# AIM-SE/AC-TSR

Hardware: NVIDIA B200
Metric: AC-SASRec train seq/s (higher is better)
Workload: dtype f32

## Files before the change

ac-tsr_b200/csrc/dense_fwd.cu:

```cuda
#include "acsr_common.cuh"
#include "../../include/acsr.h"

namespace acsr {

constexpr int kDfThreads = 352;
constexpr int kDfD = 64;
constexpr int kDfBM = 128;
constexpr int kDfOpFloats = 64 * 64;
constexpr int kDfBlkBytes = 2 * kDfOpFloats * 4;
constexpr int kDfMaxI = 256;

struct DfParams {
  const float* ctx; const float* res; long long rows, res_rows; int I, act, passes;
  const float* ops;
  const float *bo, *lnA_w, *lnA_b, *b1, *b2, *lnF_w, *lnF_b;
  float epsA, epsF, p_drop;
  const float *mask_a, *mask_f; const RngState* rng; uint32_t stream_a, stream_f;
  float *hz, *st_a, *h, *z1, *a1, *z2, *st_f, *out;
  int m_tiles;
};

__global__ void __launch_bounds__(256) dense_prep_kernel(const float* __restrict__ Wo, const float* __restrict__ W1,
                                                         const float* __restrict__ W2, int I, float* __restrict__ ops) {
  pdl_wait();
  const int nc = I / 64, blk = blockIdx.x;
  float* hi = ops + (long long)blk * 2 * kDfOpFloats;
  float* lo = hi + kDfOpFloats;
  for (int e = threadIdx.x; e < 64 * 16; e += blockDim.x) {
    const int n = e >> 4, kc = e & 15;
    const float* src;
    if (blk == 0) src = Wo + n * 64 + kc * 4;
    else if (blk <= nc) src = W1 + (long long)((blk - 1) * 64 + n) * 64 + kc * 4;
    else src = W2 + (long long)n * I + (blk - 1 - nc) * 64 + kc * 4;
    const float4 x = *reinterpret_cast<const float4*>(src);
    const float4 h4 = make_float4(to_tf32(x.x), to_tf32(x.y), to_tf32(x.z), to_tf32(x.w));
    const int off = kc * 256 + n * 4;
    *reinterpret_cast<float4*>(hi + off) = h4;
    *reinterpret_cast<float4*>(lo + off) = make_float4(x.x - h4.x, x.y - h4.y, x.z - h4.z, x.w - h4.w);
  }
}

struct DfCfg {
  static constexpr int kOffWo = 0;
  static constexpr int kOffW1 = kOffWo + kDfBlkBytes;
  static constexpr int kOffW2 = kOffW1 + 2 * kDfBlkBytes;
  static constexpr int kOffPar = kOffW2 + 2 * kDfBlkBytes;
  static constexpr int kParFloats = 6 * 64 + kDfMaxI;
  static constexpr int kOffBar = kOffPar + kParFloats * 4;
  static constexpr int kNumBars = 24;
  static constexpr int kSmemBytes = kOffBar + kNumBars * 8 + 16;
  static constexpr int kColAcc = 0, kColA = 64, kColC = 192, kColL = 320;
};

__device__ __forceinline__ float df_drop(const DfParams& p, const float* mask, uint32_t stream, long long row, int q, float* m4) {
  if (mask != nullptr) {
    const float4 mm = __ldg(reinterpret_cast<const float4*>(mask + row * kDfD + q * 4));
    m4[0] = mm.x; m4[1] = mm.y; m4[2] = mm.z; m4[3] = mm.w;
  } else if (p.p_drop > 0.f && p.rng != nullptr) {
    const float inv_keep = 1.0f / (1.0f - p.p_drop);
    const uint4 w = philox4x32(p.rng->seed, p.rng->step, stream, (unsigned long long)row * 16 + q);
    m4[0] = drop_mult(w.x, p.p_drop, inv_keep); m4[1] = drop_mult(w.y, p.p_drop, inv_keep);
    m4[2] = drop_mult(w.z, p.p_drop, inv_keep); m4[3] = drop_mult(w.w, p.p_drop, inv_keep);
  } else {
    m4[0] = m4[1] = m4[2] = m4[3] = 1.0f;
  }
  return 0.f;
}

__global__ void __launch_bounds__(kDfThreads, 1) dense_fwd_kernel(const DfParams p) {
  using Cfg = DfCfg;
  extern __shared__ __align__(128) uint8_t smem[];
  const int warp = threadIdx.x >> 5, lane = threadIdx.x & 31;
  const int nc = p.I / 64;
  float* sPar = reinterpret_cast<float*>(smem + Cfg::kOffPar);
  float *s_bo = sPar, *s_b2 = sPar + 64, *s_lnAw = sPar + 128, *s_lnAb = sPar + 192, *s_lnFw = sPar + 256, *s_lnFb = sPar + 320,
        *s_b1 = sPar + 384;
  uint64_t* bars = reinterpret_cast<uint64_t*>(smem + Cfg::kOffBar);
  uint64_t* wo_full = bars;
  uint64_t* w1_full = bars + 1;
  uint64_t* w1_empty = bars + 3;
  uint64_t* w2_full = bars + 5;
  uint64_t* w2_empty = bars + 7;
  uint64_t* a_full = bars + 9;
  uint64_t* s1_full = bars + 10;
  uint64_t* h_full = bars + 11;
  uint64_t* c_full = bars + 12;
  uint64_t* a_ready = bars + 14;
  uint64_t* c_empty = bars + 16;
  uint64_t* s3_full = bars + 18;
  uint64_t* tile_done = bars + 19;
  uint32_t* tmem_slot = reinterpret_cast<uint32_t*>(bars + Cfg::kNumBars);

  pdl_launch_dependents();
  if (threadIdx.x == 0) {
    mbar_init(wo_full, 1);
    for (int s = 0; s < 2; ++s) {
      mbar_init(w1_full + s, 1); mbar_init(w1_empty + s, 1); mbar_init(w2_full + s, 1); mbar_init(w2_empty + s, 1);
      mbar_init(c_full + s, 1); mbar_init(a_ready + s, 256); mbar_init(c_empty + s, 1);
    }
    mbar_init(a_full, 128); mbar_init(s1_full, 1); mbar_init(h_full, 128); mbar_init(s3_full, 1); mbar_init(tile_done, 128);
    mbar_fence_init();
  }
  if (warp == 1) tmem_alloc<512>(tmem_slot);
  for (int i = threadIdx.x; i < 64; i += kDfThreads) {
    s_bo[i] = p.bo[i]; s_b2[i] = p.b2[i]; s_lnAw[i] = p.lnA_w[i]; s_lnAb[i] = p.lnA_b[i]; s_lnFw[i] = p.lnF_w[i]; s_lnFb[i] = p.lnF_b[i];
  }
  for (int i = threadIdx.x; i < p.I; i += kDfThreads) s_b1[i] = p.b1[i];
  tc_fence_before();
  __syncthreads();
  tc_fence_after();
  const uint32_t tmem_base = *tmem_slot;
  const int my_tiles = (int)blockIdx.x < p.m_tiles ? (p.m_tiles - (int)blockIdx.x + (int)gridDim.x - 1) / (int)gridDim.x : 0;

  if (warp == 0) {
    if (lane == 0 && my_tiles > 0) {
      mbar_arrive_expect_tx(wo_full, kDfBlkBytes);
      bulk_g2s(smem + Cfg::kOffWo, p.ops, kDfBlkBytes, wo_full);
      for (int it = 0; it < my_tiles; ++it)
        for (int c = 0; c < nc; ++c) {
          const int g = it * nc + c, b = g & 1;
          const uint32_t ph = (g >> 1) & 1;
          mbar_wait(w1_empty + b, ph ^ 1);
          mbar_arrive_expect_tx(w1_full + b, kDfBlkBytes);
          bulk_g2s(smem + Cfg::kOffW1 + b * kDfBlkBytes, p.ops + (long long)(1 + c) * 2 * kDfOpFloats, kDfBlkBytes, w1_full + b);
          mbar_wait(w2_empty + b, ph ^ 1);
          mbar_arrive_expect_tx(w2_full + b, kDfBlkBytes);
          bulk_g2s(smem + Cfg::kOffW2 + b * kDfBlkBytes, p.ops + (long long)(1 + nc + c) * 2 * kDfOpFloats, kDfBlkBytes, w2_full + b);
        }
    }
  } else if (warp == 1 || warp == 2) {
    if (lane == 0 && my_tiles > 0) {
      const uint32_t idesc = umma_idesc_tf32(kDfBM, 64);
      constexpr uint32_t kLbo = 64 * 16, kSbo = 128;
      const int npass = p.passes == 3 ? 3 : 1;
      const uint32_t a_hi = tmem_base + Cfg::kColA, a_lo = a_hi + 64;
      auto mma24 = [&](uint32_t d_tmem, uint32_t ahi, uint32_t alo, uint32_t bsm, bool first_zero) {
        uint32_t acc = first_zero ? 0u : 1u;
        for (int ps = 0; ps < npass; ++ps) {
          const uint32_t a_base = (npass == 3 && ps == 0) ? alo : ahi;
          const uint32_t b_base = bsm + ((npass == 3 && ps == 1) ? kDfOpFloats * 4 : 0);
#pragma unroll
          for (int ks = 0; ks < 8; ++ks) {
            umma_tf32_ts(d_tmem, a_base + ks * 8, umma_desc_kmajor(b_base + ks * 2 * kLbo, kLbo, kSbo), idesc, acc);
            acc = 1;
          }
        }
      };
      if (warp == 1) {
        mbar_wait(wo_full, 0);
        for (int it = 0; it < my_tiles; ++it) {
          mbar_wait(a_full, it & 1);
          tc_fence_after();
          mma24(tmem_base + Cfg::kColAcc, a_hi, a_lo, smem_u32(smem + Cfg::kOffWo), true);
          umma_commit(s1_full);
          mbar_wait(h_full, it & 1);
          for (int c = 0; c < nc; ++c) {
            const int g = it * nc + c, b = g & 1;
            const uint32_t ph = (g >> 1) & 1;
            mbar_wait(w1_full + b, ph);
            mbar_wait(c_empty + b, ph ^ 1);
            tc_fence_after();
            mma24(tmem_base + Cfg::kColC + b * 64, a_hi, a_lo, smem_u32(smem + Cfg::kOffW1 + b * kDfBlkBytes), true);
            umma_commit(w1_empty + b);
            umma_commit(c_full + b);
          }
        }
      } else {
        for (int it = 0; it < my_tiles; ++it) {
          for (int c = 0; c < nc; ++c) {
            const int g = it * nc + c, b = g & 1;
            const uint32_t ph = (g >> 1) & 1;
            mbar_wait(a_ready + b, ph);
            mbar_wait(w2_full + b, ph);
            tc_fence_after();
            mma24(tmem_base + Cfg::kColAcc, tmem_base + Cfg::kColC + b * 64, tmem_base + Cfg::kColL + b * 64,
                  smem_u32(smem + Cfg::kOffW2 + b * kDfBlkBytes), c == 0);
            umma_commit(w2_empty + b);
            umma_commit(c_empty + b);
          }
          umma_commit(s3_full);
        }
      }
    }
  } else if (warp < 11) {
    pdl_wait();
    const int quarter = warp & 3;
    const int half = (warp - 3) >> 2;
    const int row = quarter * 32 + lane;
    const uint32_t t_lane = tmem_base + ((uint32_t)(quarter * 32) << 16);
    for (int it = 0; it < my_tiles; ++it) {
      const long long grow = (long long)(blockIdx.x + it * gridDim.x) * kDfBM + row;
      const bool row_ok = grow < p.rows;
      if (half == 1) {
        float4 cx[16];
#pragma unroll
        for (int q = 0; q < 16; ++q)
          cx[q] = row_ok ? __ldg(reinterpret_cast<const float4*>(p.ctx + grow * kDfD + q * 4)) : make_float4(0.f, 0.f, 0.f, 0.f);
        mbar_wait(tile_done, (it & 1) ^ 1);
        tc_fence_after();
#pragma unroll
        for (int hcol = 0; hcol < 2; ++hcol) {
          float hi[32], lo[32];
#pragma unroll
          for (int q = 0; q < 8; ++q) {
            const float4 v = cx[hcol * 8 + q];
            hi[4 * q] = to_tf32(v.x); hi[4 * q + 1] = to_tf32(v.y); hi[4 * q + 2] = to_tf32(v.z); hi[4 * q + 3] = to_tf32(v.w);
            lo[4 * q] = v.x - hi[4 * q]; lo[4 * q + 1] = v.y - hi[4 * q + 1]; lo[4 * q + 2] = v.z - hi[4 * q + 2]; lo[4 * q + 3] = v.w - hi[4 * q + 3];
          }
          tmem_st32(t_lane + Cfg::kColA + hcol * 32, hi);
          tmem_st32(t_lane + Cfg::kColA + 64 + hcol * 32, lo);
        }
        tc_fence_before();
        mbar_arrive(a_full);
      }
      if (half == 0) {
        mbar_wait(s1_full, it & 1);
        tc_fence_after();
        float x[64];
        tmem_ld32(t_lane + Cfg::kColAcc, x);
        tmem_ld32(t_lane + Cfg::kColAcc + 32, x + 32);
        float s = 0.f;
        if (row_ok) {
          float* hz = p.hz + grow * kDfD;
#pragma unroll
          for (int i = 0; i < 64; i += 4) *reinterpret_cast<float4*>(hz + i) = make_float4(x[i], x[i + 1], x[i + 2], x[i + 3]);
          const float* rr = p.res + (grow % p.res_rows) * kDfD;
#pragma unroll
          for (int q = 0; q < 16; ++q) {
            float m4[4];
            df_drop(p, p.mask_a, p.stream_a, grow, q, m4);
            const float4 r4 = __ldg(reinterpret_cast<const float4*>(rr + q * 4));
            const float rv[4] = {r4.x, r4.y, r4.z, r4.w};
#pragma unroll
            for (int v = 0; v < 4; ++v) {
              const int c = q * 4 + v;
              x[c] = (x[c] + s_bo[c]) * m4[v] + rv[v];
              s += x[c];
            }
          }
        } else {
#pragma unroll
          for (int c = 0; c < 64; ++c) x[c] = 0.f;
        }
        const float mean = s * (1.0f / 64);
        float var = 0.f;
#pragma unroll
        for (int c = 0; c < 64; ++c) { const float t = x[c] - mean; var = fmaf(t, t, var); }
        const float rstd = 1.0f / sqrtf(var * (1.0f / 64) + p.epsA);
#pragma unroll
        for (int c = 0; c < 64; ++c) x[c] = row_ok ? (x[c] - mean) * rstd * s_lnAw[c] + s_lnAb[c] : 0.f;
        if (row_ok) {
          float* ho = p.h + grow * kDfD;
#pragma unroll
          for (int c = 0; c < 64; c += 4) *reinterpret_cast<float4*>(ho + c) = make_float4(x[c], x[c + 1], x[c + 2], x[c + 3]);
          p.st_a[2 * grow] = mean; p.st_a[2 * grow + 1] = rstd;
        }
#pragma unroll
        for (int hcol = 0; hcol < 2; ++hcol) {
          float hi[32], lo[32];
#pragma unroll
          for (int i = 0; i < 32; ++i) { hi[i] = to_tf32(x[hcol * 32 + i]); lo[i] = x[hcol * 32 + i] - hi[i]; }
          tmem_st32(t_lane + Cfg::kColA + hcol * 32, hi);
          tmem_st32(t_lane + Cfg::kColA + 64 + hcol * 32, lo);
        }
        tc_fence_before();
        mbar_arrive(h_full);
      }
      for (int c = 0; c < nc; ++c) {
        const int g = it * nc + c, b = g & 1;
        const uint32_t ph = (g >> 1) & 1;
        mbar_wait(c_full + b, ph);
        tc_fence_after();
        float v[32], lo[32];
        tmem_ld32(t_lane + Cfg::kColC + b * 64 + half * 32, v);
        const int col0 = c * 64 + half * 32;
        if (row_ok) {
          float* z = p.z1 + grow * p.I + col0;
#pragma unroll
          for (int i = 0; i < 32; i += 4) *reinterpret_cast<float4*>(z + i) = make_float4(v[i], v[i + 1], v[i + 2], v[i + 3]);
        }
#pragma unroll
        for (int i = 0; i < 32; ++i) v[i] = row_ok ? act_fwd(p.act, v[i] + s_b1[col0 + i]) : 0.f;
        if (row_ok) {
          float* a = p.a1 + grow * p.I + col0;
#pragma unroll
          for (int i = 0; i < 32; i += 4) *reinterpret_cast<float4*>(a + i) = make_float4(v[i], v[i + 1], v[i + 2], v[i + 3]);
        }
#pragma unroll
        for (int i = 0; i < 32; ++i) { const float hi = to_tf32(v[i]); lo[i] = v[i] - hi; v[i] = hi; }
        tmem_st32(t_lane + Cfg::kColC + b * 64 + half * 32, v);
        tmem_st32(t_lane + Cfg::kColL + b * 64 + half * 32, lo);
        tc_fence_before();
        mbar_arrive(a_ready + b);
      }
      if (half == 0) {
        mbar_wait(s3_full, it & 1);
        tc_fence_after();
        float x[64];
        tmem_ld32(t_lane + Cfg::kColAcc, x);
        tmem_ld32(t_lane + Cfg::kColAcc + 32, x + 32);
        if (row_ok) {
          float* z = p.z2 + grow * kDfD;
#pragma unroll
          for (int i = 0; i < 64; i += 4) *reinterpret_cast<float4*>(z + i) = make_float4(x[i], x[i + 1], x[i + 2], x[i + 3]);
        }
        float s = 0.f;
#pragma unroll
        for (int hcol = 0; hcol < 2; ++hcol) {
          float hi[32], lo[32];
          tmem_ld32(t_lane + Cfg::kColA + hcol * 32, hi);
          tmem_ld32(t_lane + Cfg::kColA + 64 + hcol * 32, lo);
#pragma unroll
          for (int q = 0; q < 8; ++q) {
            float m4[4] = {1.f, 1.f, 1.f, 1.f};
            if (row_ok) df_drop(p, p.mask_f, p.stream_f, grow, hcol * 8 + q, m4);
#pragma unroll
            for (int v = 0; v < 4; ++v) {
              const int i = q * 4 + v, c = hcol * 32 + i;
              x[c] = (x[c] + s_b2[c]) * m4[v] + (hi[i] + lo[i]);
              s += x[c];
            }
          }
        }
        tc_fence_before();
        mbar_arrive(tile_done);
        const float mean = s * (1.0f / 64);
        float var = 0.f;
#pragma unroll
        for (int c = 0; c < 64; ++c) { const float t = x[c] - mean; var = fmaf(t, t, var); }
        const float rstd = 1.0f / sqrtf(var * (1.0f / 64) + p.epsF);
        if (row_ok) {
          float* o = p.out + grow * kDfD;
#pragma unroll
          for (int c = 0; c < 64; c += 4)
            *reinterpret_cast<float4*>(o + c) = make_float4((x[c] - mean) * rstd * s_lnFw[c] + s_lnFb[c], (x[c + 1] - mean) * rstd * s_lnFw[c + 1] + s_lnFb[c + 1],
                                                            (x[c + 2] - mean) * rstd * s_lnFw[c + 2] + s_lnFb[c + 2], (x[c + 3] - mean) * rstd * s_lnFw[c + 3] + s_lnFb[c + 3]);
          p.st_f[2 * grow] = mean; p.st_f[2 * grow + 1] = rstd;
        }
      }
    }
  }
  tc_fence_before();
  __syncthreads();
  if (warp == 1) {
    tc_fence_after();
    tmem_dealloc<512>(tmem_base);
  }
}

}

using namespace acsr;

extern "C" {

int64_t acsr_dense_prep_floats(int I) { return (I > 0 && I % 64 == 0) ? (int64_t)(1 + 2 * (I / 64)) * 2 * kDfOpFloats : 0; }

int acsr_dense_prep(const float* Wo, const float* W1, const float* W2, int d, int I, float* ops, void* stream) {
  if (d != kDfD || I <= 0 || I > kDfMaxI || (I & 63)) {
    set_error("dense_prep: hidden size %d / inner size %d unsupported (64; multiples of 64 up to %d)", d, I, kDfMaxI);
    return ACSR_ERR_UNSUPPORTED;
  }
  ACSR_REQUIRE(Wo && W1 && W2 && ops, "dense_prep: NULL pointer");
  launch_pdl(dense_prep_kernel, dim3(1 + 2 * (I / 64)), dim3(256), 0, (cudaStream_t)stream, Wo, W1, W2, I, ops);
  return check_launch("dense_prep");
}

int acsr_dense_fwd(const float* ctx, const float* res, int64_t rows, int64_t res_rows, int d, int I, int act, const float* ops,
                   const float* bo, const float* lnA_w, const float* lnA_b, float epsA, const float* b1, const float* b2,
                   const float* lnF_w, const float* lnF_b, float epsF, float p_drop, const float* mask_a, const float* mask_f,
                   const void* rng, uint32_t stream_a, uint32_t stream_f, float* hz, float* st_a, float* h, float* z1, float* a1,
                   float* z2, float* st_f, float* out, int passes, void* stream) {
  if (d != kDfD || I <= 0 || I > kDfMaxI || (I & 63)) {
    set_error("dense_fwd: hidden size %d / inner size %d unsupported (64; multiples of 64 up to %d)", d, I, kDfMaxI);
    return ACSR_ERR_UNSUPPORTED;
  }
  ACSR_REQUIRE(ctx && res && ops && bo && lnA_w && lnA_b && b1 && b2 && lnF_w && lnF_b, "dense_fwd: NULL input");
  ACSR_REQUIRE(hz && st_a && h && z1 && a1 && z2 && st_f && out, "dense_fwd: NULL output");
  ACSR_REQUIRE(rows >= 0 && res_rows > 0 && act >= 0 && act <= 4, "dense_fwd: bad sizes");
  ACSR_REQUIRE(passes == 1 || passes == 3, "dense_fwd: passes must be 1 or 3");
  ACSR_REQUIRE(p_drop >= 0.f && p_drop < 1.f, "dense_fwd: dropout p=%f", p_drop);
  ACSR_REQUIRE(!(p_drop > 0.f && rng == nullptr && (mask_a == nullptr || mask_f == nullptr)), "dense_fwd: p>0 needs masks or rng");
  if (rows == 0) return ACSR_OK;
  DfParams p = {};
  p.ctx = ctx; p.res = res; p.rows = rows; p.res_rows = res_rows; p.I = I; p.act = act; p.passes = passes; p.ops = ops;
  p.bo = bo; p.lnA_w = lnA_w; p.lnA_b = lnA_b; p.b1 = b1; p.b2 = b2; p.lnF_w = lnF_w; p.lnF_b = lnF_b;
  p.epsA = epsA; p.epsF = epsF; p.p_drop = p_drop; p.mask_a = mask_a; p.mask_f = mask_f; p.rng = (const RngState*)rng;
  p.stream_a = stream_a; p.stream_f = stream_f;
  p.hz = hz; p.st_a = st_a; p.h = h; p.z1 = z1; p.a1 = a1; p.z2 = z2; p.st_f = st_f; p.out = out;
  p.m_tiles = (int)((rows + kDfBM - 1) / kDfBM);
  static_assert(DfCfg::kSmemBytes <= 227 * 1024, "shared memory budget");
  cudaError_t e = cudaFuncSetAttribute(dense_fwd_kernel, cudaFuncAttributeMaxDynamicSharedMemorySize, DfCfg::kSmemBytes);
  if (e != cudaSuccess) { set_error("dense_fwd: smem attr: %s", cudaGetErrorString(e)); return ACSR_ERR_CUDA; }
  const int grid = p.m_tiles < kNumSMs ? p.m_tiles : kNumSMs;
  launch_pdl(dense_fwd_kernel, dim3(grid), dim3(kDfThreads), DfCfg::kSmemBytes, (cudaStream_t)stream, p);
  return check_launch("dense_fwd");
}

}
```

ac-tsr_b200/fused_step.py:

```python
import math

import torch

from . import ops
from ._lib import LIB
from .ops import _p, _stream


class _RandSlice(object):

    def __init__(self, rand, sl):
        self.rand, self.sl = rand, sl

    def get(self, key):
        t = self.rand.get(key)
        return None if t is None else t[self.sl].contiguous()


class FusedTrainStep(object):
    def __init__(self, model, optimizer):
        if model.loss_type not in ('CE', 'BPR'):
            raise NotImplementedError("Make sure 'loss_type' in ['BPR', 'CE']!")
        self.m, self.opt = model, optimizer
        self.buf = {}
        self.vp = None
        self.tc = (bool(getattr(model, 'tc_linear', True)) and model.hidden_size == 64 and model.inner_size <= 256
                   and model.inner_size % 4 == 0)
        self.tc_wgrad = bool(getattr(model, 'tc_wgrad', True))
        self.passes = 3
        self.overlap_wgrad = bool(getattr(model, 'overlap_wgrad', True))
        self.n_branches = int(getattr(model, 'step_branches', 1))
        self._streams = {}
        self.compact_last = bool(getattr(model, 'compact_last', True))
        import os
        self.order_side = os.environ.get('ACSR_ORDER_SIDE', '1') == '1'
        self.fold_attack = os.environ.get('ACSR_FOLD_ATTACK', '1') == '1'
        self.fold_gate = os.environ.get('ACSR_FOLD_GATE', '0') == '1'
        self.pdl = bool(getattr(model, 'pdl', True))
        self.tail_fused = (self.tc and model.inner_size % 16 == 0 and os.environ.get('ACSR_TAIL_FUSED', '1') == '1')
        self.fuse_act_bwd = os.environ.get('ACSR_FUSE_ACT_BWD', '0') == '1'
        self.dense_fused = (self.tc and model.inner_size % 64 == 0 and os.environ.get('ACSR_DENSE_FUSED', '0') == '1')
        self.dense_bwd = (self.tc and model.inner_size % 64 == 0 and os.environ.get('ACSR_DENSE_BWD', '1') == '1')
        self.split_wgrad = int(os.environ.get('ACSR_SPLIT_WGRAD', '1'))
        self.ce_fused_bwd = model.hidden_size == 64 and os.environ.get('ACSR_CE_FUSED_BWD', '1') == '1'

    def _stream_for(self, dev, key):
        if key not in self._streams:
            self._streams[key] = torch.cuda.Stream(device=dev)
        return self._streams[key]

    def _branch_buffers(self, Bs, L, dev, idx, grads=True):
        key = ('branch', Bs, L, idx)
        if key in self.buf:
            return self.buf[key]
        m = self.m
        d, I, N = m.hidden_size, m.inner_size, m.n_layers
        T = Bs * L

        def f(*s):
            return torch.empty(s, dtype=torch.float32, device=dev)
        b = dict(T=T, x0=f(T, d), st_e=f(T, 2), layers=[], order=torch.empty(Bs, dtype=torch.int32, device=dev))
        for l in range(N):
            R = 2 * T if l == N - 1 else T
            qkv5 = f(6, T, d)
            qkv, aqk = qkv5[:3], qkv5[3:5]
            Rp = 1 if (l == N - 1 and self.compact_last) else R
            lb = dict(qkv5=qkv5, qkv=qkv, aqk=aqk, mq=qkv[0], mk=qkv[1], mv=qkv[2], aq=aqk[0], ak=aqk[1],
                      gl=(qkv5[5].view(-1)[:T * L].view(T, L) if L <= d else f(T, L)), ctx=f(R, d),
                      hz=f(Rp, d), st_a=f(Rp, 2), h=f(Rp, d), z1=f(Rp, I), a1=f(Rp, I), z2=f(Rp, d), st_f=f(Rp, 2), out=f(Rp, d))
            if grads:
                for n, w in (('d_z2', d), ('d_z1', I), ('d_hz', d), ('d_gl', L)):
                    lb[n] = f(2 * T if (Rp > 1 or n == 'd_gl') else 1, w)
                lb['d_qkv'], lb['d_aqk'] = f(3, 2 * T, d), f(2, 2 * T, d)
                lb['d_mq'], lb['d_mk'], lb['d_mv'] = lb['d_qkv'][0], lb['d_qkv'][1], lb['d_qkv'][2]
                lb['d_aq'], lb['d_ak'] = lb['d_aqk'][0], lb['d_aqk'][1]
            b['layers'].append(lb)
        C = 2 * Bs
        b['c'] = dict(ctx=f(C, d), x=f(Bs, d), hz=f(C, d), st_a=f(C, 2), h=f(C, d), z1=f(C, I), a1=f(C, I), z2=f(C, d), st_f=f(C, 2),
                      out=f(C, d), d_out=f(C, d), d_z2=f(C, d), d_h=f(C, d), d_a1=f(C, I), d_z1=f(C, I), d_hz=f(C, d), d_x=f(C, d),
                      d_ctx=f(C, d))
        if grads:
            for n, w in (('d_out', d), ('d_a1', I), ('d_h', d), ('d_x', d), ('d_ctx', d)):
                b[n] = f(2 * T, w)
        self.buf[key] = b
        return b

    def _joint_buffers(self, B, dev):
        key = ('joint', B)
        if key in self.buf:
            return self.buf[key]
        m = self.m
        d, N, V = m.hidden_size, m.n_layers, m.n_items

        def f(*s):
            return torch.empty(s, dtype=torch.float32, device=dev)
        nc = ops.logits_num_chunks(2 * B, V, d)
        loss3 = f(3)
        j = dict(pen=torch.zeros(N, dtype=torch.float64, device=dev), out2=f(2 * B, d), partial=f(2 * B, nc, 2), lse=f(2 * B),
                 tgt=f(2 * B), row_loss=f(2 * B), loss3=loss3, loss=loss3[:2], loss_att=loss3[2:], dpen=f(N), Gt=None,
                 d_out2=f(2 * B, d),
                 target2=torch.empty(2 * B, dtype=torch.int64, device=dev), ce_cnt=torch.zeros(1, dtype=torch.int32, device=dev),
                 neg2=torch.empty(2 * B, dtype=torch.int64, device=dev), row_x=f(2 * B),
                 row_scale=torch.cat((torch.full((B,), 1.0 / B), torch.full((B,), -1.0 / B))).to(dev))
        self.buf[key] = j
        return j

    @torch.no_grad()
    def __call__(self, interaction):
        was = LIB.query('acsr_set_pdl', 1 if self.pdl else 0)
        try:
            return self._step(interaction)
        finally:
            LIB.query('acsr_set_pdl', was)

    def _step(self, interaction):
        m, opt = self.m, self.opt
        seq = interaction[m.ITEM_SEQ].contiguous()
        ln = interaction[m.ITEM_SEQ_LEN].contiguous()
        pos_items = interaction[m.POS_ITEM_ID]
        B, L = seq.shape
        dev = seq.device
        d, N, V = m.hidden_size, m.n_layers, m.n_items
        rt = m._runtime(dev)
        rng, rand = rt.rng, rt.rand
        training = m.training
        E = m.item_embedding.weight
        main = torch.cuda.current_stream()
        nb = self.n_branches if (self.n_branches > 1 and B % self.n_branches == 0 and L <= 64 and self.vp is None) else 1
        Bs = B // nb
        jb = self._joint_buffers(B, dev)
        branches = []
        for s in range(nb):
            sl = slice(s * Bs, (s + 1) * Bs)
            branches.append(dict(idx=s, sl=sl, seq=seq[sl], ln=ln[sl], buf=self._branch_buffers(Bs, L, dev, s),
                                 rand=rand if (rand is None or nb == 1) else _RandSlice(rand, sl),
                                 stream=main if s == 0 else self._stream_for(dev, ('branch', s)),
                                 side=self._stream_for(dev, ('side', s)) if self.overlap_wgrad else None))
        rng.advance()
        jb['pen'].zero_()
        torch.cat((pos_items, pos_items), out=jb['target2'])
        zero_done = None
        if training:
            zs = self._stream_for(dev, ('zero',))
            zs.wait_stream(main)
            with torch.cuda.stream(zs):
                opt.zero_grad()
                jb['d_out2'].zero_()
                for br in branches:
                    bb = br['buf']
                    if self._sharded():
                        self._shard_buffers(bb, dev)['d_xrows'].zero_()
                    if self.compact_last:
                        bb['d_ctx'].zero_()
                        bb['d_x'].zero_()
                    else:
                        bb['d_out'].zero_()
                    for l, layer in enumerate(m.trm_encoder.layer):
                        if layer.combine_option == 'gate':
                            bb['layers'][l]['d_gl'].zero_()
            zero_done = torch.cuda.Event()
            zero_done.record(zs)
        for br in branches:
            if br['stream'] is not main:
                br['stream'].wait_stream(main)
            with torch.cuda.stream(br['stream']):
                self._forward_branch(br, jb, B, L, rt, training)
        for br in branches:
            if br['stream'] is not main:
                main.wait_stream(br['stream'])
        if getattr(self, '_stop_after', None) == 'fwd':
            if zero_done is not None:
                main.wait_event(zero_done)
            return jb['loss'][0], jb['loss'][0]
        st = _stream()
        passes = m.logits_passes
        vst = None
        if self.vp is not None:
            loss2, vst = self.vp.ce_forward(jb['out2'], E, jb['target2'], 2)
            jb['loss'].copy_(loss2)
        wp = m.mask_loss_weight.detach() if m.trainable_mask_loss_weight else None
        wv = 0.0 if wp is not None else float(m.mask_loss_weight)
        bpr = m.loss_type == 'BPR'
        if bpr:
            if self.vp is not None:
                raise NotImplementedError('vocab-parallel logits are a CE construct; loss_type BPR touches two table rows per sequence')
            neg_items = interaction[m.NEG_ITEM_ID]
            torch.cat((neg_items, neg_items), out=jb['neg2'])
            LIB.call('acsr_bpr_loss_fwd', _p(jb['out2']), _p(E), _p(jb['target2'], torch.int64), _p(jb['neg2'], torch.int64), 2 * B, d, 2,
                     float(m.loss_fct.gamma), _p(jb['row_x']), _p(jb['row_loss']), _p(jb['loss']), st)
            LIB.call('acsr_loss_combine', jb['pen'].data_ptr(), N, _p(jb['loss'][1:]), _p(wp), wv, _p(jb['loss_att']), _p(jb['dpen']), st)
        elif self.vp is None:
            LIB.call('acsr_logits_ce_partial', _p(jb['out2']), _p(E), 2 * B, V, d, passes, _p(jb['partial']), st)
            LIB.call('acsr_ce_finalize_losses', _p(jb['partial']), jb['partial'].shape[1], _p(jb['out2']), _p(E),
                     _p(jb['target2'], torch.int64), 2 * B, d, V, 0, 2, _p(jb['lse']), _p(jb['tgt']), _p(jb['row_loss']),
                     _p(jb['loss']), jb['pen'].data_ptr(), N, _p(wp), wv, _p(jb['loss_att']), _p(jb['dpen']),
                     jb['ce_cnt'].data_ptr(), st)
        else:
            LIB.call('acsr_loss_combine', jb['pen'].data_ptr(), N, _p(jb['loss'][1:]), _p(wp), wv, _p(jb['loss_att']), _p(jb['dpen']), st)
        loss_cal = jb['loss'][0]
        loss_att = jb['loss_att'][0]
        self.last_losses = jb['loss3']
        if not training or getattr(self, '_stop_after', None) == 'ce':
            if zero_done is not None:
                main.wait_event(zero_done)
            return loss_att, loss_cal
        dpen = jb['dpen']
        main.wait_event(zero_done)
        if bpr:
            LIB.call('acsr_bpr_loss_bwd', _p(jb['out2']), _p(E), _p(jb['target2'], torch.int64), _p(jb['neg2'], torch.int64),
                     _p(jb['row_x']), _p(jb['row_scale']), 2 * B, d, float(m.loss_fct.gamma), 0, B, _p(jb['d_out2']), _p(E.grad), st)
        elif self.vp is not None:
            jb['d_out2'].copy_(self.vp.ce_backward(vst, E, jb['row_scale'], E.grad, table_half=0, n_groups=2))
        elif self.ce_fused_bwd:
            ops.ce_bwd_dout(jb['out2'], E, jb['lse'], jb['target2'], jb['row_scale'], jb['d_out2'], passes)
        else:
            if jb['Gt'] is None:
                jb['Gt'] = torch.empty((V, 2 * B), dtype=torch.float32, device=dev)
            LIB.call('acsr_logits_ce_grad', _p(jb['out2']), _p(E), _p(jb['lse']), _p(jb['target2'], torch.int64),
                     _p(jb['row_scale']), 2 * B, V, d, passes, _p(jb['Gt']), 2 * B, st)
            if self.tc_wgrad:
                ops.gemm_batch([ops.wgrad_problem(jb['Gt'], E, V, 2 * B, d, jb['d_out2'])])
            else:
                LIB.call('acsr_linear_wgrad', _p(jb['Gt']), _p(E), V, 2 * B, d, _p(jb['d_out2']), None, st)
        for br in branches:
            if br['stream'] is not main:
                br['stream'].wait_stream(main)
        if self.vp is None and not bpr:
            dE_stream = branches[0]['side'] if (nb == 1 and branches[0]['side'] is not None) else main
            if dE_stream is not main:
                dE_stream.wait_stream(main)
            with torch.cuda.stream(dE_stream):
                if self.ce_fused_bwd:
                    ops.ce_bwd_dtable(jb['out2'][:B], E, jb['lse'][:B], jb['target2'][:B], jb['row_scale'][:B], E.grad, passes)
                elif self.tc and B <= 256:
                    ops.linear_tok(jb['Gt'], V, B, jb['out2'], d, E.grad, d, ldx=2 * B, w_sn=1, w_sk=d, wkb=64 * d, accumulate=True)
                else:
                    ops.gemm_batch([ops.gemm_problem(jb['Gt'], jb['out2'], E.grad, V, d, B, a_strides=(2 * B, 1, 0, B),
                                                     b_strides=(1, d, 0, B), accumulate=True)])
        else:
            dE_stream = main
        dE_done = torch.cuda.Event()
        dE_done.record(dE_stream)
        for br in branches:
            with torch.cuda.stream(br['stream']):
                self._backward_branch(br, jb, B, L, rt, dpen, dE_done)
        for br in branches:
            if br['stream'] is not main:
                main.wait_stream(br['stream'])
        return loss_att, loss_cal

    def _forward_branch(self, br, jb, B, L, rt, training, need_att=True):
        m = self.m
        b, seq, ln, s = br['buf'], br['seq'], br['ln'], br['idx']
        Bs = seq.shape[0]
        T, d, I, N, V, H = b['T'], m.hidden_size, m.inner_size, m.n_layers, m.n_items, m.n_heads
        dh = d // H
        rng, rand = rt.rng, br['rand']
        rngp = rng.ptr
        st = _stream()
        p_h = m.dropout.p if training else 0.0
        soff = 4096 * s

        def mask(key):
            return None if (rand is None or p_h == 0.0) else rand.get(key)

        def mask2(l, k_cal, k_att, last):
            if rand is None or p_h == 0.0:
                return None
            a = rand.get((l, k_cal))
            return torch.cat((a.reshape(T, d), rand.get((l, k_att)).reshape(T, d))) if last else a

        E = m.item_embedding.weight
        posw = m.position_embedding.weight if m.use_position_embedding else None
        b['me'] = mask('emb')
        cur = torch.cuda.current_stream()
        so = self._stream_for(seq.device, ('order', s)) if self.order_side else cur
        if so is not cur:
            so.wait_stream(cur)
        folded = {}
        if self.tc and self.fold_attack:
            for l in range(N):
                st3 = self._stacked(l)
                if st3 is None:
                    continue
                fw = self._folded_buffers(l, seq.device)
                lay = m.trm_encoder.layer[l]
                fw['gate'] = lay.combine_option == 'gate' and lay.gate.out_features == L and L <= d and self.fold_gate
                LIB.call('acsr_fold_projection_weights', _p(st3['Wqkv']), _p(st3['bqkv']), _p(st3['Waqk']), _p(st3['baqk']), d,
                         _p(lay.gate.weight) if fw['gate'] else None, _p(lay.gate.bias) if fw['gate'] else None, L if fw['gate'] else 0,
                         _p(fw['W']), _p(fw['b']), so.cuda_stream)
                fw['done'] = torch.cuda.Event()
                fw['done'].record(so)
                folded[l] = fw
        dense_ops = {}
        if self.dense_fused:
            for l in range(N):
                if l == N - 1 and self.compact_last and self.tail_fused:
                    continue
                lay = m.trm_encoder.layer[l]
                dbuf = self._dense_ops_buffer(l, seq.device)
                LIB.call('acsr_dense_prep', _p(lay.attack_attention.dense.weight), _p(lay.feed_forward.dense_1.weight),
                         _p(lay.feed_forward.dense_2.weight), d, I, _p(dbuf['ops']), so.cuda_stream)
                dbuf['done'] = torch.cuda.Event()
                dbuf['done'].record(so)
                dense_ops[l] = dbuf
        b['dense_ops'] = dense_ops
        bwd_ops = {}
        if self.dense_bwd and training and not self.fuse_act_bwd:
            for l in range(N):
                if l == N - 1 and self.compact_last and self.tail_fused:
                    continue
                lay = m.trm_encoder.layer[l]
                dbuf = self._dense_bwd_ops_buffer(l, s, seq.device)
                LIB.call('acsr_dense_bwd_prep', _p(lay.attack_attention.dense.weight), _p(lay.feed_forward.dense_1.weight),
                         _p(lay.feed_forward.dense_2.weight), d, I, _p(dbuf), so.cuda_stream)
                bwd_ops[l] = dbuf
        b['dense_bwd_ops'] = bwd_ops
        LIB.call('acsr_seq_order', _p(seq, torch.int64), Bs, L, _p(b['order'], torch.int32), so.cuda_stream)
        order_done = torch.cuda.Event()
        order_done.record(so)
        if self._sharded():
            sb = self._shard_buffers(b, seq.device)
            _, b['ids_all'] = self.vp.fetch_rows(seq.reshape(-1), E, out=sb['xrows'][1:])
            LIB.call('acsr_embed_ln_dropout_fwd', _p(sb['iota1'], torch.int64), _p(sb['xrows']), _p(posw), _p(m.LayerNorm.weight),
                     _p(m.LayerNorm.bias), m.LayerNorm.eps, T, L, d, T + 1, p_h, _p(b['me']), rngp, soff + 1, _p(b['x0']), _p(b['st_e']), st)
        else:
            LIB.call('acsr_embed_ln_dropout_fwd', _p(seq, torch.int64), _p(E), _p(posw), _p(m.LayerNorm.weight), _p(m.LayerNorm.bias),
                     m.LayerNorm.eps, T, L, d, V, p_h, _p(b['me']), rngp, soff + 1, _p(b['x0']), _p(b['st_e']), st)
        x = b['x0']
        b['xs'] = []
        act_id = ops.ACT_IDS[m.hidden_act]
        for l, layer in enumerate(m.trm_encoder.layer):
            last = l == N - 1 and need_att
            R = 2 * T if last else T
            lb = b['layers'][l]
            aa, ff = layer.attack_attention, layer.feed_forward
            base = soff + 16 * (l + 1)
            b['xs'].append(x)
            st3 = self._stacked(l)
            if l in folded and so is not cur:
                cur.wait_event(folded[l]['done'])
            if st3 is not None and self.tc and self.fold_attack:
                fw = folded[l]
                if fw['gate']:
# ... 384 lines not shown
```

Before: 408,300.

## Rework fused dense forward epilogue and enable it by default

Restructures the epilogue warps of the fused attention-output/FFN dense forward kernel. Each row is now split across two warps by column half, with a shared-memory exchange for the LayerNorm row sums. Global loads and stores are staged through shared memory so they coalesce. The next tile's context is prefetched into tensor memory while the current tile finishes, which removes the tile_done barrier. The activation function is dispatched through templates, the weight load skips the PDL wait when the weights are static, and the fused path becomes the default. This replaces separate dense kernels with one fused kernel, at the cost of more shared memory, extra named barriers and the correctness risk of a new fused path.

Result: faster. 432,000 (median of 6 runs) (+5.8%).

```diff
diff --git a/ac-tsr_b200/csrc/dense_fwd.cu b/ac-tsr_b200/csrc/dense_fwd.cu
--- a/ac-tsr_b200/csrc/dense_fwd.cu
+++ b/ac-tsr_b200/csrc/dense_fwd.cu
@@ -9,6 +9,7 @@
 constexpr int kDfOpFloats = 64 * 64;
 constexpr int kDfBlkBytes = 2 * kDfOpFloats * 4;
 constexpr int kDfMaxI = 256;
+constexpr int kDfStgPitch = 36;
 
 struct DfParams {
   const float* ctx; const float* res; long long rows, res_rows; int I, act, passes;
@@ -17,7 +18,7 @@
   float epsA, epsF, p_drop;
   const float *mask_a, *mask_f; const RngState* rng; uint32_t stream_a, stream_f;
   float *hz, *st_a, *h, *z1, *a1, *z2, *st_f, *out;
-  int m_tiles;
+  int m_tiles, w_static;
 };
 
 __global__ void __launch_bounds__(256) dense_prep_kernel(const float* __restrict__ Wo, const float* __restrict__ W1,
@@ -46,25 +47,90 @@
   static constexpr int kOffW2 = kOffW1 + 2 * kDfBlkBytes;
   static constexpr int kOffPar = kOffW2 + 2 * kDfBlkBytes;
   static constexpr int kParFloats = 6 * 64 + kDfMaxI;
-  static constexpr int kOffBar = kOffPar + kParFloats * 4;
+  static constexpr int kOffStg = kOffPar + kParFloats * 4;
+  static constexpr int kStgFloats = 32 * kDfStgPitch;
+  static constexpr int kOffXch = kOffStg + 8 * kStgFloats * 4;
+  static constexpr int kOffBar = kOffXch + 4 * 2 * kDfBM * 4;
   static constexpr int kNumBars = 24;
   static constexpr int kSmemBytes = kOffBar + kNumBars * 8 + 16;
   static constexpr int kColAcc = 0, kColA = 64, kColC = 192, kColL = 320;
 };
 
-__device__ __forceinline__ float df_drop(const DfParams& p, const float* mask, uint32_t stream, long long row, int q, float* m4) {
-  if (mask != nullptr) {
-    const float4 mm = __ldg(reinterpret_cast<const float4*>(mask + row * kDfD + q * 4));
-    m4[0] = mm.x; m4[1] = mm.y; m4[2] = mm.z; m4[3] = mm.w;
-  } else if (p.p_drop > 0.f && p.rng != nullptr) {
+__device__ __forceinline__ void df_drop32(const DfParams& p, const float* mask, uint32_t stream, long long row, int c0, bool ok,
+                                          float* m) {
+  if (!ok || (mask == nullptr && !(p.p_drop > 0.f && p.rng != nullptr))) {
+#pragma unroll
+    for (int i = 0; i < 32; ++i) m[i] = 1.0f;
+  } else if (mask != nullptr) {
+#pragma unroll
+    for (int q = 0; q < 8; ++q) {
+      const float4 mm = __ldg(reinterpret_cast<const float4*>(mask + row * kDfD + c0) + q);
+      m[4 * q] = mm.x; m[4 * q + 1] = mm.y; m[4 * q + 2] = mm.z; m[4 * q + 3] = mm.w;
+    }
+  } else {
     const float inv_keep = 1.0f / (1.0f - p.p_drop);
-    const uint4 w = philox4x32(p.rng->seed, p.rng->step, stream, (unsigned long long)row * 16 + q);
-    m4[0] = drop_mult(w.x, p.p_drop, inv_keep); m4[1] = drop_mult(w.y, p.p_drop, inv_keep);
-    m4[2] = drop_mult(w.z, p.p_drop, inv_keep); m4[3] = drop_mult(w.w, p.p_drop, inv_keep);
-  } else {
-    m4[0] = m4[1] = m4[2] = m4[3] = 1.0f;
-  }
-  return 0.f;
+    const unsigned long long seed = p.rng->seed, step = p.rng->step;
+#pragma unroll
+    for (int q = 0; q < 8; ++q) {
+      const uint4 w = philox4x32(seed, step, stream, (unsigned long long)row * 16 + (c0 >> 2) + q);
+      m[4 * q] = drop_mult(w.x, p.p_drop, inv_keep); m[4 * q + 1] = drop_mult(w.y, p.p_drop, inv_keep);
+      m[4 * q + 2] = drop_mult(w.z, p.p_drop, inv_keep); m[4 * q + 3] = drop_mult(w.w, p.p_drop, inv_keep);
+    }
+  }
+}
+
+__device__ __forceinline__ void df_load32(float* stg, const float* src, long long ld, long long row0, long long rows, long long mod,
+                                          int lane, float* v) {
+  const int c = 4 * (lane & 7);
+  float4 x[8];
+#pragma unroll
+  for (int i = 0; i < 8; ++i) {
+    const long long g = row0 + 4 * i + (lane >> 3);
+    x[i] = g < rows ? __ldg(reinterpret_cast<const float4*>(src + (g < mod ? g : g % mod) * ld + c)) : make_float4(0.f, 0.f, 0.f, 0.f);
+  }
+#pragma unroll
+  for (int i = 0; i < 8; ++i) *reinterpret_cast<float4*>(stg + (4 * i + (lane >> 3)) * kDfStgPitch + c) = x[i];
+  __syncwarp();
+#pragma unroll
+  for (int q = 0; q < 8; ++q) {
+    const float4 y = *reinterpret_cast<const float4*>(stg + lane * kDfStgPitch + 4 * q);
+    v[4 * q] = y.x; v[4 * q + 1] = y.y; v[4 * q + 2] = y.z; v[4 * q + 3] = y.w;
+  }
+  __syncwarp();
+}
+
+__device__ __forceinline__ void df_store32(float* stg, float* dst, long long ld, long long row0, long long rows, int lane, const float* v) {
+#pragma unroll
+  for (int q = 0; q < 8; ++q)
+    *reinterpret_cast<float4*>(stg + lane * kDfStgPitch + 4 * q) = make_float4(v[4 * q], v[4 * q + 1], v[4 * q + 2], v[4 * q + 3]);
+  __syncwarp();
+  const int c = 4 * (lane & 7);
+#pragma unroll
+  for (int i = 0; i < 8; ++i) {
+    const int r = 4 * i + (lane >> 3);
+    if (row0 + r < rows) *reinterpret_cast<float4*>(dst + (row0 + r) * ld + c) = *reinterpret_cast<const float4*>(stg + r * kDfStgPitch + c);
+  }
+  __syncwarp();
+}
+
+__device__ __forceinline__ void df_store_split(uint32_t taddr, uint32_t lo_off, float* v, float* lo) {
+#pragma unroll
+  for (int i = 0; i < 32; ++i) { const float hi = to_tf32(v[i]); lo[i] = v[i] - hi; v[i] = hi; }
+  tmem_st32(taddr, v);
+  tmem_st32(taddr + lo_off, lo);
+}
+
+__device__ __forceinline__ float df_row_sum(float v, float* xch, int half, int row, int quarter) {
+  xch[half * kDfBM + row] = v;
+  asm volatile("bar.sync %0, 64;" ::"r"(1 + quarter) : "memory");
+  const float o = xch[(half ^ 1) * kDfBM + row];
+  return half == 0 ? v + o : o + v;
+}
+
+template <int ACT>
+__device__ __forceinline__ void df_act32(float* v, const float* b, bool ok) {
+#pragma unroll
+  for (int i = 0; i < 32; ++i) v[i] = ok ? act_fwd(ACT, v[i] + b[i]) : 0.f;
 }
 
 __global__ void __launch_bounds__(kDfThreads, 1) dense_fwd_kernel(const DfParams p) {
@@ -88,7 +154,6 @@
   uint64_t* a_ready = bars + 14;
   uint64_t* c_empty = bars + 16;
   uint64_t* s3_full = bars + 18;
-  uint64_t* tile_done = bars + 19;
   uint32_t* tmem_slot = reinterpret_cast<uint32_t*>(bars + Cfg::kNumBars);
 
   pdl_launch_dependents();
@@ -98,7 +163,7 @@
       mbar_init(w1_full + s, 1); mbar_init(w1_empty + s, 1); mbar_init(w2_full + s, 1); mbar_init(w2_empty + s, 1);
       mbar_init(c_full + s, 1); mbar_init(a_ready + s, 256); mbar_init(c_empty + s, 1);
     }
-    mbar_init(a_full, 128); mbar_init(s1_full, 1); mbar_init(h_full, 128); mbar_init(s3_full, 1); mbar_init(tile_done, 128);
+    mbar_init(a_full, 256); mbar_init(s1_full, 1); mbar_init(h_full, 256); mbar_init(s3_full, 1);
     mbar_fence_init();
   }
   if (warp == 1) tmem_alloc<512>(tmem_slot);
@@ -114,6 +179,7 @@
 
   if (warp == 0) {
     if (lane == 0 && my_tiles > 0) {
+      if (!p.w_static) pdl_wait();
       mbar_arrive_expect_tx(wo_full, kDfBlkBytes);
       bulk_g2s(smem + Cfg::kOffWo, p.ops, kDfBlkBytes, wo_full);
       for (int it = 0; it < my_tiles; ++it)
@@ -182,161 +248,118 @@
         }
       }
     }
-  } else if (warp < 11) {
+  } else {
     pdl_wait();
     const int quarter = warp & 3;
     const int half = (warp - 3) >> 2;
+    const int c0 = half * 32;
     const int row = quarter * 32 + lane;
     const uint32_t t_lane = tmem_base + ((uint32_t)(quarter * 32) << 16);
+    float* stg = reinterpret_cast<float*>(smem + Cfg::kOffStg) + (warp - 3) * Cfg::kStgFloats;
+    float* xch = reinterpret_cast<float*>(smem + Cfg::kOffXch);
+    auto ctx_to_tmem = [&](int it) {
+      float v[32], lo[32];
+      df_load32(stg, p.ctx + c0, kDfD, (long long)(blockIdx.x + it * gridDim.x) * kDfBM + quarter * 32, p.rows, p.rows, lane, v);
+      df_store_split(t_lane + Cfg::kColA + c0, 64, v, lo);
+    };
+    if (my_tiles > 0) {
+      ctx_to_tmem(0);
+      tc_fence_before();
+      mbar_arrive(a_full);
+    }
     for (int it = 0; it < my_tiles; ++it) {
-      const long long grow = (long long)(blockIdx.x + it * gridDim.x) * kDfBM + row;
+      const long long row0 = (long long)(blockIdx.x + it * gridDim.x) * kDfBM + quarter * 32;
+      const long long grow = row0 + lane;
       const bool row_ok = grow < p.rows;
-      if (half == 1) {
-        float4 cx[16];
-#pragma unroll
-        for (int q = 0; q < 16; ++q)
-          cx[q] = row_ok ? __ldg(reinterpret_cast<const float4*>(p.ctx + grow * kDfD + q * 4)) : make_float4(0.f, 0.f, 0.f, 0.f);
-        mbar_wait(tile_done, (it & 1) ^ 1);
-        tc_fence_after();
-#pragma unroll
-        for (int hcol = 0; hcol < 2; ++hcol) {
-          float hi[32], lo[32];
-#pragma unroll
-          for (int q = 0; q < 8; ++q) {
-            const float4 v = cx[hcol * 8 + q];
-            hi[4 * q] = to_tf32(v.x); hi[4 * q + 1] = to_tf32(v.y); hi[4 * q + 2] = to_tf32(v.z); hi[4 * q + 3] = to_tf32(v.w);
-            lo[4 * q] = v.x - hi[4 * q]; lo[4 * q + 1] = v.y - hi[4 * q + 1]; lo[4 * q + 2] = v.z - hi[4 * q + 2]; lo[4 * q + 3] = v.w - hi[4 * q + 3];
-          }
-          tmem_st32(t_lane + Cfg::kColA + hcol * 32, hi);
-          tmem_st32(t_lane + Cfg::kColA + 64 + hcol * 32, lo);
-        }
-        tc_fence_before();
-        mbar_arrive(a_full);
-      }
-      if (half == 0) {
+      const bool next = it + 1 < my_tiles;
+      {
+        float r[32], m[32], x[32];
+        df_load32(stg, p.res + c0, kDfD, row0, p.rows, p.res_rows, lane, r);
+        df_drop32(p, p.mask_a, p.stream_a, grow, c0, row_ok, m);
         mbar_wait(s1_full, it & 1);
         tc_fence_after();
-        float x[64];
-        tmem_ld32(t_lane + Cfg::kColAcc, x);
-        tmem_ld32(t_lane + Cfg::kColAcc + 32, x + 32);
+        tmem_ld32(t_lane + Cfg::kColAcc + c0, x);
+        df_store32(stg, p.hz + c0, kDfD, row0, p.rows, lane, x);
         float s = 0.f;
-        if (row_ok) {
-          float* hz = p.hz + grow * kDfD;
-#pragma unroll
-          for (int i = 0; i < 64; i += 4) *reinterpret_cast<float4*>(hz + i) = make_float4(x[i], x[i + 1], x[i + 2], x[i + 3]);
-          const float* rr = p.res + (grow % p.res_rows) * kDfD;
-#pragma unroll
-          for (int q = 0; q < 16; ++q) {
-            float m4[4];
-            df_drop(p, p.mask_a, p.stream_a, grow, q, m4);
-            const float4 r4 = __ldg(reinterpret_cast<const float4*>(rr + q * 4));
-            const float rv[4] = {r4.x, r4.y, r4.z, r4.w};
-#pragma unroll
-            for (int v = 0; v < 4; ++v) {
-              const int c = q * 4 + v;
-              x[c] = (x[c] + s_bo[c]) * m4[v] + rv[v];
-              s += x[c];
-            }
-          }
-        } else {
-#pragma unroll
-          for (int c = 0; c < 64; ++c) x[c] = 0.f;
-        }
-        const float mean = s * (1.0f / 64);
+#pragma unroll
+        for (int i = 0; i < 32; ++i) {
+          x[i] = (x[i] + s_bo[c0 + i]) * m[i] + r[i];
+          s += x[i];
+        }
+        const float mean = df_row_sum(s, xch, half, row, quarter) * (1.0f / 64);
         float var = 0.f;
 #pragma unroll
-        for (int c = 0; c < 64; ++c) { const float t = x[c] - mean; var = fmaf(t, t, var); }
+        for (int i = 0; i < 32; ++i) { const float t = x[i] - mean; var = fmaf(t, t, var); }
+        var = df_row_sum(var, xch + 2 * kDfBM, half, row, quarter);
         const float rstd = 1.0f / sqrtf(var * (1.0f / 64) + p.epsA);
 #pragma unroll
-        for (int c = 0; c < 64; ++c) x[c] = row_ok ? (x[c] - mean) * rstd * s_lnAw[c] + s_lnAb[c] : 0.f;
-        if (row_ok) {
-          float* ho = p.h + grow * kDfD;
-#pragma unroll
-          for (int c = 0; c < 64; c += 4) *reinterpret_cast<float4*>(ho + c) = make_float4(x[c], x[c + 1], x[c + 2], x[c + 3]);
-          p.st_a[2 * grow] = mean; p.st_a[2 * grow + 1] = rstd;
-        }
-#pragma unroll
-        for (int hcol = 0; hcol < 2; ++hcol) {
-          float hi[32], lo[32];
-#pragma unroll
-          for (int i = 0; i < 32; ++i) { hi[i] = to_tf32(x[hcol * 32 + i]); lo[i] = x[hcol * 32 + i] - hi[i]; }
-          tmem_st32(t_lane + Cfg::kColA + hcol * 32, hi);
-          tmem_st32(t_lane + Cfg::kColA + 64 + hcol * 32, lo);
-        }
+        for (int i = 0; i < 32; ++i) x[i] = row_ok ? (x[i] - mean) * rstd * s_lnAw[c0 + i] + s_lnAb[c0 + i] : 0.f;
+        df_store_split(t_lane + Cfg::kColA + c0, 64, x, r);
         tc_fence_before();
         mbar_arrive(h_full);
+#pragma unroll
+        for (int i = 0; i < 32; ++i) x[i] += r[i];
+        df_store32(stg, p.h + c0, kDfD, row0, p.rows, lane, x);
+        if (half == 0 && row_ok) { p.st_a[2 * grow] = mean; p.st_a[2 * grow + 1] = rstd; }
       }
       for (int c = 0; c < nc; ++c) {
         const int g = it * nc + c, b = g & 1;
         const uint32_t ph = (g >> 1) & 1;
+        const int col0 = c * 64 + c0;
         mbar_wait(c_full + b, ph);
         tc_fence_after();
         float v[32], lo[32];
-        tmem_ld32(t_lane + Cfg::kColC + b * 64 + half * 32, v);
-        const int col0 = c * 64 + half * 32;
-        if (row_ok) {
-          float* z = p.z1 + grow * p.I + col0;
-#pragma unroll
-          for (int i = 0; i < 32; i += 4) *reinterpret_cast<float4*>(z + i) = make_float4(v[i], v[i + 1], v[i + 2], v[i + 3]);
-        }
-#pragma unroll
-        for (int i = 0; i < 32; ++i) v[i] = row_ok ? act_fwd(p.act, v[i] + s_b1[col0 + i]) : 0.f;
-        if (row_ok) {
-          float* a = p.a1 + grow * p.I + col0;
-#pragma unroll
-          for (int i = 0; i < 32; i += 4) *reinterpret_cast<float4*>(a + i) = make_float4(v[i], v[i + 1], v[i + 2], v[i + 3]);
-        }
-#pragma unroll
-        for (int i = 0; i < 32; ++i) { const float hi = to_tf32(v[i]); lo[i] = v[i] - hi; v[i] = hi; }
-        tmem_st32(t_lane + Cfg::kColC + b * 64 + half * 32, v);
-        tmem_st32(t_lane + Cfg::kColL + b * 64 + half * 32, lo);
+        tmem_ld32(t_lane + Cfg::kColC + b * 64 + c0, v);
+        df_store32(stg, p.z1 + col0, p.I, row0, p.rows, lane, v);
+        switch (p.act) {
+          case ACT_GELU: df_act32<ACT_GELU>(v, s_b1 + col0, row_ok); break;
+          case ACT_RELU: df_act32<ACT_RELU>(v, s_b1 + col0, row_ok); break;
+          case ACT_SWISH: df_act32<ACT_SWISH>(v, s_b1 + col0, row_ok); break;
+          case ACT_TANH: df_act32<ACT_TANH>(v, s_b1 + col0, row_ok); break;
+          default: df_act32<ACT_SIGMOID>(v, s_b1 + col0, row_ok); break;
+        }
+        df_store_split(t_lane + Cfg::kColC + b * 64 + c0, Cfg::kColL - Cfg::kColC, v, lo);
         tc_fence_before();
         mbar_arrive(a_ready + b);
+#pragma unroll
+        for (int i = 0; i < 32; ++i) v[i] += lo[i];
+        df_store32(stg, p.a1 + col0, p.I, row0, p.rows, lane, v);
       }
-      if (half == 0) {
+      {
+        float hs[32], m[32], x[32];
+        {
+          float lo[32];
+          tmem_ld32(t_lane + Cfg::kColA + c0, hs);
+          tmem_ld32(t_lane + Cfg::kColA + 64 + c0, lo);
+#pragma unroll
+          for (int i = 0; i < 32; ++i) hs[i] += lo[i];
+        }
+        if (next) ctx_to_tmem(it + 1);
+        df_drop32(p, p.mask_f, p.stream_f, grow, c0, row_ok, m);
         mbar_wait(s3_full, it & 1);
         tc_fence_after();
-        float x[64];
-        tmem_ld32(t_lane + Cfg::kColAcc, x);
-        tmem_ld32(t_lane + Cfg::kColAcc + 32, x + 32);
-        if (row_ok) {
-          float* z = p.z2 + grow * kDfD;
-#pragma unroll
-          for (int i = 0; i < 64; i += 4) *reinterpret_cast<float4*>(z + i) = make_float4(x[i], x[i + 1], x[i + 2], x[i + 3]);
-        }
+        tmem_ld32(t_lane + Cfg::kColAcc + c0, x);
+        if (next) {
+          tc_fence_before();
+          mbar_arrive(a_full);
+        }
+        df_store32(stg, p.z2 + c0, kDfD, row0, p.rows, lane, x);
         float s = 0.f;
 #pragma unroll
-        for (int hcol = 0; hcol < 2; ++hcol) {
-          float hi[32], lo[32];
-          tmem_ld32(t_lane + Cfg::kColA + hcol * 32, hi);
-          tmem_ld32(t_lane + Cfg::kColA + 64 + hcol * 32, lo);
-#pragma unroll
-          for (int q = 0; q < 8; ++q) {
-            float m4[4] = {1.f, 1.f, 1.f, 1.f};
-            if (row_ok) df_drop(p, p.mask_f, p.stream_f, grow, hcol * 8 + q, m4);
-#pragma unroll
-            for (int v = 0; v < 4; ++v) {
-              const int i = q * 4 + v, c = hcol * 32 + i;
-              x[c] = (x[c] + s_b2[c]) * m4[v] + (hi[i] + lo[i]);
-              s += x[c];
-            }
-          }
-        }
-        tc_fence_before();
-        mbar_arrive(tile_done);
-        const float mean = s * (1.0f / 64);
+        for (int i = 0; i < 32; ++i) {
+          x[i] = (x[i] + s_b2[c0 + i]) * m[i] + hs[i];
+          s += x[i];
+        }
+        const float mean = df_row_sum(s, xch + 4 * kDfBM, half, row, quarter) * (1.0f / 64);
         float var = 0.f;
 #pragma unroll
-        for (int c = 0; c < 64; ++c) { const float t = x[c] - mean; var = fmaf(t, t, var); }
+        for (int i = 0; i < 32; ++i) { const float t = x[i] - mean; var = fmaf(t, t, var); }
+        var = df_row_sum(var, xch + 6 * kDfBM, half, row, quarter);
         const float rstd = 1.0f / sqrtf(var * (1.0f / 64) + p.epsF);
-        if (row_ok) {
-          float* o = p.out + grow * kDfD;
-#pragma unroll
-          for (int c = 0; c < 64; c += 4)
-            *reinterpret_cast<float4*>(o + c) = make_float4((x[c] - mean) * rstd * s_lnFw[c] + s_lnFb[c], (x[c + 1] - mean) * rstd * s_lnFw[c + 1] + s_lnFb[c + 1],
-                                                            (x[c + 2] - mean) * rstd * s_lnFw[c + 2] + s_lnFb[c + 2], (x[c + 3] - mean) * rstd * s_lnFw[c + 3] + s_lnFb[c + 3]);
-          p.st_f[2 * grow] = mean; p.st_f[2 * grow + 1] = rstd;
-        }
+#pragma unroll
+        for (int i = 0; i < 32; ++i) x[i] = (x[i] - mean) * rstd * s_lnFw[c0 + i] + s_lnFb[c0 + i];
+        df_store32(stg, p.out + c0, kDfD, row0, p.rows, lane, x);
+        if (half == 0 && row_ok) { p.st_f[2 * grow] = mean; p.st_f[2 * grow + 1] = rstd; }
       }
     }
   }
@@ -389,6 +412,7 @@
   p.stream_a = stream_a; p.stream_f = stream_f;
   p.hz = hz; p.st_a = st_a; p.h = h; p.z1 = z1; p.a1 = a1; p.z2 = z2; p.st_f = st_f; p.out = out;
   p.m_tiles = (int)((rows + kDfBM - 1) / kDfBM);
+  p.w_static = is_static_memory(ops);
   static_assert(DfCfg::kSmemBytes <= 227 * 1024, "shared memory budget");
   cudaError_t e = cudaFuncSetAttribute(dense_fwd_kernel, cudaFuncAttributeMaxDynamicSharedMemorySize, DfCfg::kSmemBytes);
   if (e != cudaSuccess) { set_error("dense_fwd: smem attr: %s", cudaGetErrorString(e)); return ACSR_ERR_CUDA; }
diff --git a/ac-tsr_b200/fused_step.py b/ac-tsr_b200/fused_step.py
--- a/ac-tsr_b200/fused_step.py
+++ b/ac-tsr_b200/fused_step.py
@@ -39,7 +39,7 @@
         self.pdl = bool(getattr(model, 'pdl', True))
         self.tail_fused = (self.tc and model.inner_size % 16 == 0 and os.environ.get('ACSR_TAIL_FUSED', '1') == '1')
         self.fuse_act_bwd = os.environ.get('ACSR_FUSE_ACT_BWD', '0') == '1'
-        self.dense_fused = (self.tc and model.inner_size % 64 == 0 and os.environ.get('ACSR_DENSE_FUSED', '0') == '1')
+        self.dense_fused = (self.tc and model.inner_size % 64 == 0 and os.environ.get('ACSR_DENSE_FUSED', '1') == '1')
         self.dense_bwd = (self.tc and model.inner_size % 64 == 0 and os.environ.get('ACSR_DENSE_BWD', '1') == '1')
         self.split_wgrad = int(os.environ.get('ACSR_SPLIT_WGRAD', '1'))
         self.ce_fused_bwd = model.hidden_size == 64 and os.environ.get('ACSR_CE_FUSED_BWD', '1') == '1'
```
